# Roman-HLIS-Cosmology-PIT/romanimpreprocess

Measured on AMD Instinct MI355X. Metric: SCA ramps/sec (4096x4096x8grp full L1->L2 chain), higher is better.
Workload: dtype f32

## Files before the change

### romanimpreprocess_amd/csrc/chain2_form.h

```cpp
#pragma once
#include "rip_common.h"

constexpr int c2_block(int n, int want) {
    int d = want < 1 ? 1 : want;
    while (n % d) --d;
    return d;
}
template <int G, bool K64>
struct C2Form {
    static_assert(G % 2 == 0 && G > 4 && G <= 16, "forms exist for whole pairs of groups, 6 to 16");
    static constexpr int narrow = G > 8 ? 2 : (K64 ? 1 : 0);
    static constexpr int cols = (narrow == 0 || (narrow == 2 && K64)) ? 256 : 384;
    static constexpr int threads = 2 * cols;
    static constexpr int outw = cols - 4;
    static constexpr int nstrips(int nx) { return (nx - 4 + outw - 1) / outw < 1 ? 1 : (nx - 4 + outw - 1) / outw; }
    static constexpr int wps = narrow == 0 ? 4 : ((narrow == 2 && K64) ? 2 : 3);

    static constexpr int ks = K64 ? 8 : 4;
    static constexpr int x_ofs = 0;
    static constexpr int o1_ofs = x_ofs + G / 2 * 3 * cols * 8;
    static constexpr int dq_ofs = o1_ofs + G * 3 * cols * ks;
    static constexpr bool wring = narrow < 2;
    static constexpr int qs_ofs = dq_ofs + 3 * cols * 4;
    static constexpr int gn_ofs = qs_ofs + (wring ? 3 * ((G + 3) / 4) * cols * 4 : 0);
    static constexpr int nlc = cols / RIP_CW + 1;
    static constexpr int ln_ofs = gn_ofs + (wring ? 3 * cols * 4 : 0);
    static constexpr int kr_ofs = ln_ofs + nlc * G * 2 * 8;
    static constexpr int krn_room = (160 * 1024 - kr_ofs) / (2 * cols * ks);
    static constexpr int krn = narrow == 2 ? 0 : (krn_room < 9 ? krn_room : 9);
    static constexpr int lds_bytes = kr_ofs + 2 * krn * cols * ks;
    static_assert(lds_bytes <= (narrow == 0 ? 80 : 160) * 1024, "the 256-column form runs two workgroups per CU, the others one");

    static constexpr int stream_aux = narrow == 2 ? 2 : 0;
    static constexpr int pb = c2_block(G / 2, narrow == 2 ? (K64 ? 4 : 1) : 2);
    static constexpr int pbc = c2_block(G / 2, wps == 2 ? 2 : 1);
    static constexpr int nbo = c2_block(G, G > 8 ? 4 : 2);
    static_assert((G / 2) % pb == 0 && (G / 2) % pbc == 0 && G % nbo == 0, "block factors divide their counts");
};

static inline long chain2_geometry(ChainArgs &a, int nstrips, int live_last, int slots, int reserve, int wc = 4, bool quad_ok = true) {
    const int maxr = (a.ny + 7) / 8;
    auto cdiv = [](int x, int y) { return (x + y - 1) / y; };
    int best_nr = 0, best_nq = 0, best_steps = 1 << 30;
    if (quad_ok && nstrips > 1 && live_last <= 64) {
        const int nfull = nstrips - 1;
        for (int pass = 0; pass < 2 && !best_nr; ++pass) {
            const int avail = slots - (pass ? 0 : reserve);
            for (int nq = 1; wc * nq <= maxr && nq < avail; ++nq) {
                int nr = (avail - nq) / nfull;
                if (nr > maxr) nr = maxr;
                if (nr < 1) break;
                const int steps = cdiv(a.ny, nr) > cdiv(a.ny, wc * nq) ? cdiv(a.ny, nr) : cdiv(a.ny, wc * nq);
                if (steps < best_steps) best_steps = steps, best_nr = nr, best_nq = nq;
            }
        }
    }
    int nr_u = (slots - reserve) / nstrips;
    if (nr_u < 1) nr_u = slots / nstrips;
    if (nr_u > maxr) nr_u = maxr;
    if (nr_u < 1) nr_u = 1;
    if (best_nr && best_steps < cdiv(a.ny, nr_u)) {
        a.geo_nr = best_nr, a.geo_rows = cdiv(a.ny, best_nr), a.geo_nq = best_nq, a.geo_rows_q = cdiv(a.ny, wc * best_nq);
        return (long)best_nr * (nstrips - 1) + best_nq;
// ... 20 lines not shown
```

### romanimpreprocess_amd/csrc/chain2_kernel.h

```cpp
#pragma once
#include "chain_common.h"
#include "chain2_form.h"

#if (defined(C2_DBG) || defined(CH_STAMP)) && !defined(RIP_TIMING_BUILD)
#error "C2_DBG / CH_STAMP are timing experiments: build them with -DRIP_TIMING_BUILD"
#endif
#ifdef CH_STAMP
#define C2_DRAIN()                                \
    if (a.dbg & 2048) {                           \
        __builtin_amdgcn_s_waitcnt(0);            \
    }
#else
#define C2_DRAIN()
#endif
#define C2_SYNC() __syncthreads()

__device__ __forceinline__ unsigned c2_opaque(unsigned x) {
    asm volatile("" : "+v"(x));
    return x;
}

__device__ __forceinline__ __amdgpu_buffer_rsrc_t c2_rsrc(const void *p, int records = -1) {
    return __builtin_amdgcn_make_buffer_rsrc(const_cast<void *>(p), 0, records, 0x00020000);
}
// ... 58 lines not shown
    static_assert(NA >= NG && G0 >= 0 && G0 < NG, "the values G0 .. NG - 1 of NA are divided");
    const double b = (double)bf;
    double y = __builtin_amdgcn_rcp(b);
    double e = __builtin_fma(-b, y, 1.0);
    y = __builtin_fma(y, e, y);
    e = __builtin_fma(-b, y, 1.0);
    y = __builtin_fma(y, e, y);
    float asum = 0.0f, amin = 3.0e38f;
#pragma unroll
    for (int g = G0; g < NG; ++g) {
        const double q0 = a[g] * y;
        const double r = __builtin_fma(-b, q0, a[g]);
        qf[g] = (float)__builtin_fma(r, y, q0);
        asum = asum + fabsf(qf[g]);
        amin = fminf(amin, fabsf(qf[g]));
    }
    const bool ok = rcp_safe(bf) && asum < 5.7e17f && amin > 1.8e-18f;
    if (!__all(ok || !use)) {
#pragma unroll
        for (int g = G0; g < NG; ++g) qf[g] = (float)(a[g] / b);
    }
}

template <int NP>
struct C2Legendre {
    const float (&cfs)[NP], (&c1s)[NP], (&c2s)[NP], (&chfs)[NP];
    static constexpr __device__ int n() { return NP; }
    __device__ __forceinline__ float cf(int L) const { return cfs[L]; }
    __device__ __forceinline__ float c1(int L) const { return c1s[L]; }
    __device__ __forceinline__ float c2(int L) const { return c2s[L]; }
    __device__ __forceinline__ float chf(int L) const { return chfs[L]; }
};

template <int NP, int G, int START, typename KT, bool SKIP0 = false>
__global__ __launch_bounds__((C2Form<G + (G & 1), sizeof(KT) == 8>::threads), (C2Form<G + (G & 1), sizeof(KT) == 8>::wps)) void chain2_kernel(
    ChainArgs a, const RipPlanHeader *__restrict__ h, const RipVariant *__restrict__ vars, const float *__restrict__ kvals,
    const RipDiff *__restrict__ diffs, double guard) {
    static_assert(G > 4 && G <= 16, "pairs of groups; the groupdq bytes travel packed four to a word");
    static_assert(!SKIP0 || START == 1, "group 0 can be skipped only where the fit excludes it");
    constexpr int GE = G + (G & 1);
    using F = C2Form<GE, sizeof(KT) == 8>;
    constexpr int COLS = F::cols;
    constexpr int KRN = F::krn;
    constexpr bool KFIT = F::narrow > 0;
    constexpr int QW = (G + 3) / 4;
    constexpr int GP = GE / 2;
    static_assert(QW == (GE + 3) / 4, "the padded count packs into the same flag words");
    constexpr bool K64 = sizeof(KT) == 8;
    constexpr int SA = F::stream_aux;
    extern __shared__ __align__(16) unsigned char lds_raw[];
    constexpr int XR = 3;
    f2 *X2 = reinterpret_cast<f2 *>(lds_raw + F::x_ofs);
    f2 *O12 = reinterpret_cast<f2 *>(lds_raw + F::o1_ofs);
    double *O1d = reinterpret_cast<double *>(lds_raw + F::o1_ofs);
    uint32_t *DQ = reinterpret_cast<uint32_t *>(lds_raw + F::dq_ofs);
    uint32_t *QS = reinterpret_cast<uint32_t *>(lds_raw + F::qs_ofs);
    float *GN = reinterpret_cast<float *>(lds_raw + F::gn_ofs);
    double *LN = reinterpret_cast<double *>(lds_raw + F::ln_ofs);
    constexpr int NLC = F::nlc;
    f2 *KR2 = reinterpret_cast<f2 *>(lds_raw + F::kr_ofs);
    float *KR1 = reinterpret_cast<float *>(KR2 + 2 * 4 * COLS);
    double *KRd = reinterpret_cast<double *>(lds_raw + F::kr_ofs);

    const RIP_K C2KernArgs *kargs = (const RIP_K C2KernArgs *)__builtin_amdgcn_kernarg_segment_ptr();
    const int tid = threadIdx.x;
    if (a.wg_counter && tid == 0) __hip_atomic_fetch_add(a.wg_counter, 1u, __ATOMIC_RELAXED, __HIP_MEMORY_SCOPE_AGENT);
#ifdef C2_DBG
    const int dbg = a.dbg;
#else
    constexpr int dbg = 0;
#endif
    const bool fit_role = tid >= COLS;
    const int col = fit_role ? tid - COLS : tid;
    const int ny = a.ny, nx = a.nx, nb = a.nb;
    const int ay0 = nb, ay1 = ny - nb, ax0 = nb, ax1 = nx - nb;
    const unsigned npix = (unsigned)ny * (unsigned)nx;
    const unsigned pl4 = npix * 4u;
    const int nch = nx / RIP_CW;
    const uint32_t bad = DQ_NO_LIN_CORR | DQ_REFERENCE_PIXEL;

    float c1[NP], c2[NP], chf[NP];
#pragma unroll
    for (int L = 1; L < NP; ++L) {
        const RipLegendreK k = rip_legendre_k(L);
        c1[L] = k.c1, c2[L] = k.c2, chf[L] = k.chf;
    }

    const int nstrips = F::nstrips(nx);
    const int bid = c2_xcd_block((int)blockIdx.x, (int)gridDim.x);
    const int nfull = a.geo_rows_q ? nstrips - 1 : nstrips;
    const bool quad = bid >= nfull * a.geo_nr;
// ... 59 lines not shown
            rok[dyi] = sy >= ay0 && sy < ay1;
            rowoff[dyi] = (unsigned)min(max(sy, ylo), yhi) * (row4 * ES);
        }
        const unsigned rowbits = rip_ipc_row_mask(rok[0], rok[1], rok[2]);
        const __amdgpu_buffer_rsrc_t kr = c2_rsrc(kern_base);
        unsigned pofs = 0;
#pragma unroll
        for (int p = 0; p < 9; ++p) {
            const int dy = p / 3 - 1, dx = p % 3 - 1;
            const int k = rip_ipc_term(dy, dx);
            if constexpr (PAIRS) {
                const float kv_ = c2_ld_f32(kr, cx4[dx + 1], pofs + rowoff[dy + 1]);
                if (k & 1)
                    kk[k / 2].y = kv_;
                else
                    kk[k / 2].x = kv_;
            } else {
                if (k >= KMIN) kk[k] = c2_ld_f64(kr, cx4[dx + 1] * 2u, pofs + rowoff[dy + 1]);
            }
            pofs += pl4 * ES;
        }
        const unsigned um = (want && y >= ay0 && y < ay1) ? rowbits : 0u;
        return lane_mask & um;
    };
    auto k_valid = [&](int y) -> unsigned {
        const bool r0 = (y + 1) >= ay0 && (y + 1) < ay1, r1 = y >= ay0 && y < ay1, r2 = (y - 1) >= ay0 && (y - 1) < ay1;
        return r1 ? (lane_mask & rip_ipc_row_mask(r0, r1, r2)) : 0u;
    };
#ifdef CH_STAMP
    unsigned long long st_[9] = {0, 0, 0, 0, 0, 0, 0, 0, 0};
    unsigned long long tl_ = __builtin_amdgcn_s_memtime();
#endif
    if (!fit_role) {
        auto fetch_groups = [&](const RIP_K ChainArgs *ka, int y, int g0, int g1, RowRegs<NP, GE> &rr) {
            if ((dbg & 64) && y > R0 - 2) return;
            __builtin_amdgcn_sched_barrier(0);
            const unsigned yl = (unsigned)min(max(y, ylo), yhi);
            const __amdgpu_buffer_rsrc_t rs = c2_rsrc(ka->data), rq = c2_rsrc(ka->gdq), rd = c2_rsrc(ka->dark_data),
                                         rb = c2_rsrc(ka->bias, ka->bias_records);
            unsigned o4 = yl * row4 + (unsigned)g0 * pl4, o2 = yl * (row4 >> 1) + (unsigned)g0 * (pl4 >> 1),
                     o1 = yl * (row4 >> 2) + (unsigned)g0 * npix;
#pragma unroll
            for (int g = g0; g < g1; ++g) {
                if constexpr (GE > G) {
                    if (g >= G) continue;
                }
                const bool flags_only = SKIP0 && g == 0;
                if (!flags_only) rr.S[g] = c2_ld_u16<SA>(rs, cc2, o2);
                rr.q[g] = c2_ld_u8<F::wring ? SA : 0>(rq, cc1, o1);
                if (!flags_only) {
                    rr.dk[g] = c2_ld_f32<SA>(rd, cc4, o4);
                    rr.bs[g] = c2_ld_f32<SA>(rb, cc4, o4);
                }
                o4 += pl4;
                o2 += pl4 >> 1;
                o1 += npix;
            }
            __builtin_amdgcn_sched_barrier(0);
        };
        auto fetch_coefs = [&](const RIP_K ChainArgs *ka, int y, int i0, int i1, RowRegs<NP, GE> &rr) {
            if ((dbg & 64) && y > R0 - 2) return;
            __builtin_amdgcn_sched_barrier(0);
            const unsigned yl = (unsigned)min(max(y, ylo), yhi);
            const __amdgpu_buffer_rsrc_t rp = c2_rsrc(ka->planes);
            unsigned o4 = yl * row4 + (unsigned)i0 * pl4;
#pragma unroll
            for (int i = i0; i < i1; ++i) {
                if (i < NP)
                    rr.cf[i] = c2_ld_f32<SA>(rp, cc4, o4);
                else if (i == NP)
                    rr.smin = c2_ld_f32<SA>(rp, cc4, o4);
                else if (i == NP + 1)
                    rr.smax = c2_ld_f32<SA>(rp, cc4, o4);
                else if (i == NP + 2)
                    rr.sref = c2_ld_f32<SA>(rp, cc4, o4);
                else if (i == NP + 3)
                    rr.dq = c2_ld_u32<SA>(rp, cc4, yl * row4 + (unsigned)(NP + ka->merged_dq) * pl4);
                else
                    rr.gain = c2_ld_f32<F::wring ? SA : 0>(rp, cc4, o4);
                o4 += pl4;
            }
            __builtin_amdgcn_sched_barrier(0);
        };
        auto fetch_row = [&](int y, RowRegs<NP, GE> &rr) {
            const RIP_K ChainArgs *ka = &kargs->a;
            fetch_coefs(ka, y, 0, NP + 5, rr);
            fetch_groups(ka, y, 0, G, rr);
        };
        constexpr int NCO = NP + 5;
        constexpr int CO_STEP = (NCO + GP - 1) / GP;
        RowRegs<NP, GE> rr;
        if constexpr (GE > G) rr.S[G] = rr.q[G] = 0u, rr.dk[G] = rr.bs[G] = 0.0f;
        if constexpr (SKIP0) rr.S[0] = 0u, rr.dk[0] = rr.bs[0] = 0.0f;
        fetch_row(R0 - 2, rr);
        int so_c = (R0 - 5 + 2 + 3000) % 3;
        double rcn[G];
        {
            const RIP_K double *rt = rip_k(kargs->a.rowcorr_t) + (size_t)min(max(R0 - 2, 0), ny - 1) * G;
#pragma unroll
            for (int g = SKIP0 ? 1 : 0; g < G; ++g) rcn[g] = rt[g];
            if constexpr (SKIP0) rcn[0] = 0.0;
        }
        for (int r = R0 - 5; r <= R0 + rows_wg; ++r, so_c = (so_c == 2) ? 0 : so_c + 1) {
            const RIP_K ChainArgs *ka = &c2_args(kargs)->a;
            const int yi = r + 3, yc = r + 2;
            const bool do_a = (yi >= R0 - 2) && (yi <= R1 + 1);
            const bool do_c = (yc >= R0 - 1) && (yc <= R1);
            double rc[G];
#pragma unroll
            for (int g = 0; g < G; ++g) rc[g] = rcn[g];
            {
                const RIP_K double *rt = rip_k(ka->rowcorr_t) + (size_t)min(max(yi + 1, 0), ny - 1) * G;
#pragma unroll
                for (int g = SKIP0 ? 1 : 0; g < G; ++g) rcn[g] = rt[g];
            }
            const bool a_full = do_a && yi >= 0 && yi < ny;
            const int xslot = (so_c == 2) ? 0 : so_c + 1;
            f2 *xs = X2 + xslot * COLS + col;
            const bool act = col_act && yi >= ay0 && yi < ay1;
            uint32_t dq = rr.dq;
            uint32_t w[QW];
#pragma unroll
            for (int i = 0; i < QW; ++i) w[i] = 0;
            const float smin = rr.smin;
            const float span = rr.smax - smin;
            const bool fastdiv = __all(rcp_safe(span));
            const float rspan = rip_rcp_mid(span);
            const double yd = (double)yi;
            constexpr int PB = F::pb;
#pragma unroll
            for (int pb = 0; pb < GP; pb += PB) {
                f2 zz[PB], SS[PB];
                bool any_ex = false;
                if (a_full && !(dbg & 32)) {
                    f2 tt[PB], quo[PB];
#pragma unroll
                    for (int b = 0; b < PB; ++b) {
                        const int p = pb + b;
                        float Sv[2];
#pragma unroll
                        for (int e = 0; e < 2; ++e) {
                            const int g = 2 * p + e;
                            if constexpr (GE > G) {
                                if (g >= G) {
                                    Sv[e] = Sv[0];
                                    continue;
                                }
                            }
                            if constexpr (SKIP0) {
                                if (g == 0) {
                                    w[0] |= rr.q[0] & 0xffu;
                                    continue;
                                }
                            }
                            const double *ln = LN + (chr * G + g) * 2;
                            float S = rip_refpix_apply((float)rr.S[g], rr.dk[g], rc[g], ln[0], ln[1], yd);
                            if (act) S = S - rr.bs[g];
                            Sv[e] = S;
                            w[g / 4] |= (rr.q[g] & 0xffu) << (8 * (g & 3));
                        }
                        if constexpr (SKIP0) {
                            if (p == 0) Sv[0] = Sv[1];
                        }
                        SS[b] = f2{Sv[0], Sv[1]};
                        const f2 t = SS[b] - f2{smin, smin};
                        tt[b] = t * 2.0f;
                    }
                    if (fastdiv) {
#pragma unroll
                        for (int b = 0; b < PB; ++b) quo[b] = div_rcp2(tt[b], span, rspan);
                    } else {
#pragma unroll
                        for (int b = 0; b < PB; ++b) quo[b] = f2{tt[b].x / span, tt[b].y / span};
                    }
#pragma unroll
                    for (int b = 0; b < PB; ++b) {
                        f2 z = quo[b] + (-1.0f);
                        if constexpr (!SKIP0) {
                            if (pb + b == 0 && a.do_not_flag_first) z.x = clip2<float>(z.x, -1.0f, 1.0f);
                        }
                        zz[b] = z;
                        any_ex = any_ex || (fabsf(z.x) > 1.0f) || (fabsf(z.y) > 1.0f);
                    }
                } else {
#pragma unroll
                    for (int b = 0; b < PB; ++b) zz[b] = SS[b] = f2{0.0f, 0.0f};
                }
                fetch_groups(ka, r + 4, 2 * pb, 2 * (pb + PB), rr);
                if (a_full && (dbg & 16)) {
#pragma unroll
// ... 74 lines not shown
                        if constexpr (SKIP0) {
                            if (p == 0) xv.x = 0.0f;
                        }
                        xs[p * XR * COLS] = col_ok ? xv : f2{0.0f, 0.0f};
                    }
                } else if (do_a) {
#pragma unroll
                    for (int b = 0; b < PB; ++b) xs[(pb + b) * XR * COLS] = f2{0.0f, 0.0f};
                }
            }
            if (do_a) {
                const bool keep = a_full && col_ok;
                DQ[xslot * COLS + col] = keep ? dq : 0u;
                if constexpr (F::wring) {
#pragma unroll
                    for (int i = 0; i < QW; ++i) QS[(xslot * QW + i) * COLS + col] = keep ? w[i] : 0u;
                    GN[xslot * COLS + col] = rr.gain;
                }
            }
            f2 kC[5];
            double kCd[9];
            kC[4].y = 0.0f;
            unsigned vC;
            if constexpr (K64)
                vC = load_k(ka->kern, yc, do_c && wcol >= 1 && wcol < wl - 1, kCd, C2Int<0>{});
            else
                vC = load_k(ka->kern, yc, do_c && wcol >= 1 && wcol < wl - 1, kC, C2Int<0>{});
            CH_T(2)
            C2_SYNC();
            CH_T(3)
            const RIP_K ChainArgs *kb2 = &c2_args(kargs)->a;
            auto fetch_coefs_beside = [&](int p) { fetch_coefs(kb2, r + 4, p * CO_STEP, min(p * CO_STEP + CO_STEP, NCO), rr); };
            CH_T(4)
            {
                const bool all = __all(vC == 0x1ffu || vC == 0u);
                const int so = so_c;
                const int sm = (so == 0) ? 2 : so - 1, s0 = so, sp = (so == 2) ? 0 : so + 1;
                if constexpr (KRN > 0) {
                    const int ks = yc & 1;
                    if constexpr (K64) {
#pragma unroll
                        for (int k = 0; k < KRN; ++k) KRd[(ks * KRN + k) * COLS + col] = kCd[k];
                    } else {
#pragma unroll
                        for (int i = 0; i < 4; ++i) KR2[(ks * 4 + i) * COLS + col] = kC[i];
                        KR1[ks * COLS + col] = kC[4].x;
                    }
                }
                if constexpr (K64) {
                    constexpr int PBC = F::pbc;
#pragma unroll
                    for (int p0 = 0; p0 < GP; p0 += PBC) {
#pragma unroll
                        for (int q = 0; q < PBC; ++q)
                            fetch_coefs_beside(p0 + q);
                        if (do_c) {
                            float v[2 * PBC][9];
#pragma unroll
                            for (int q = 0; q < PBC; ++q) {
                                const f2 *xb = X2 + (p0 + q) * XR * COLS + col;
                                const f2 *xm_ = xb + sm * COLS, *x0_ = xb + s0 * COLS, *xp_ = xb + sp * COLS;
                                const f2 tt[9] = {x0_[0], xm_[0], xp_[0], x0_[-1], x0_[1], xm_[-1], xm_[1], xp_[-1], xp_[1]};
#pragma unroll
                                for (int k = 0; k < 9; ++k) v[2 * q][k] = tt[k].x, v[2 * q + 1][k] = tt[k].y;
                            }
                            double f[2 * PBC];
// ... 318 lines not shown
                    for (int i = 0; i < QW; ++i) qw_next[i] = QS[(sn * QW + i) * COLS + col];
                    gain_next = GN[sn * COLS + col];
                } else {
                    const unsigned yl = (unsigned)min(max((dbg & 1024) ? R0 : r + 1, ylo), yhi);
                    const __amdgpu_buffer_rsrc_t rq = c2_rsrc(kg->a.gdq);
                    unsigned o1 = yl * (row4 >> 2);
#pragma unroll
                    for (int g = 0; g < G; ++g) {
                        qb_next[g] = c2_ld_u8(rq, cc1, o1);
                        o1 += npix;
                    }
                    gain_next = c2_ld_f32(c2_rsrc(kg->a.planes), cc4, (unsigned)(NP + 4) * pl4 + yl * row4);
                }
            }
            if constexpr (KFIT) {
                if constexpr (K64)
                    (void)load_k(kg->a.kern, (dbg & 1024) ? R0 : r + 1, true, kn_d, C2Int<KRN>{});
                else
                    (void)load_k(kg->a.kern, (dbg & 1024) ? R0 : r + 1, true, kn, C2Int<0>{});
            }
            CH_T(6)
            C2_SYNC();
            CH_T(7)
        }
    }
#ifdef CH_STAMP
    if ((tid & 63) == 0 && a.dbg_buf) {
        unsigned long long *o = a.dbg_buf + ((size_t)blockIdx.x * (F::threads / 64) + (tid >> 6)) * 9;
        for (int i = 0; i < 9; ++i) o[i] += st_[i];
    }
#endif
}

template <int NP, int G, int START, typename KT, bool SKIP0 = false>
static int launch_chain2_s(rip_ctx *ctx, const RipPlan *plan, const ChainArgs &a) {
    using F = C2Form<G + (G & 1), sizeof(KT) == 8>;
    const size_t lds = F::lds_bytes;
    if (a.nb < 2) return 1;
    ChainArgs ag = a;
    const long grid = c2_form_geometry<F>(ag, ctx->ncu, ctx->chain_reserve, ctx->chain_quad, ctx->last_geo);
    static bool lds_set[64] = {};
    if (lds > 48 * 1024 && !lds_set[ctx->device & 63]) {
        RIP_HIP(ctx, hipFuncSetAttribute(reinterpret_cast<const void *>(chain2_kernel<NP, G, START, KT, SKIP0>),
                                         hipFuncAttributeMaxDynamicSharedMemorySize, (int)lds));
        lds_set[ctx->device & 63] = true;
    }
    hipLaunchKernelGGL((chain2_kernel<NP, G, START, KT, SKIP0>), dim3((unsigned)grid), dim3(F::threads), lds, ctx->stream, ag,
                       reinterpret_cast<const RipPlanHeader *>(plan->dev), plan->d_variants, plan->d_k, plan->d_diffs,
                       ctx->guard_band);
    RIP_HIP(ctx, hipGetLastError());
    if (ag.wg_counter) ctx->gate_total += (uint32_t)grid, ctx->gate_armed = true;
    return RIP_OK;
}

template <int NP, int G, typename KT>
static int launch_chain2(rip_ctx *ctx, const RipPlan *plan, const ChainArgs &a, bool skip0) {
    if (plan->h.start == 0 && plan->dense.valid == rip_full_valid<G, 0>()) return skip0 ? 1 : launch_chain2_s<NP, G, 0, KT>(ctx, plan, a);
    if (plan->h.start == 1 && plan->dense.valid == rip_full_valid<G, 1>())
        return skip0 ? launch_chain2_s<NP, G, 1, KT, true>(ctx, plan, a) : launch_chain2_s<NP, G, 1, KT>(ctx, plan, a);
    return 1;
}

template <int NP, typename KT, int PART>
int rip_launch_chain2(rip_ctx *ctx, const RipPlan *plan, const ChainArgs &a, bool skip0) {
    static_assert(PART >= 0 && PART <= 2, "parts of RIP_CHAIN_G_ALL");
#define C2_CASE(g) \
    if (a.ngrp == g) return launch_chain2<NP, g, KT>(ctx, plan, a, skip0);
    if constexpr (PART == 0) {
        RIP_CHAIN_G_PART0(C2_CASE)
    } else if constexpr (PART == 1) {
        RIP_CHAIN_G_PART1(C2_CASE)
    } else {
        RIP_CHAIN_G_PART2(C2_CASE)
    }
#undef C2_CASE
    return 1;
}
```

### romanimpreprocess_amd/csrc/chain_common.h

```cpp
#pragma once
#include "rip_common.h"

#include "device_rampfit.h"

#ifdef CH_STAMP
#define CH_T(i)                                                     \
    {                                                               \
        const unsigned long long t_ = __builtin_amdgcn_s_memtime(); \
        __builtin_amdgcn_s_waitcnt(0xC07F);                         \
        st_[i] += t_ - tl_;                                         \
        tl_ = t_;                                                   \
    }
#else
#define CH_T(i)
#endif

typedef float f2 __attribute__((ext_vector_type(2)));

__device__ __forceinline__ f2 div_rcp2(f2 a, float b, float rb) {
    const f2 nb = {-b, -b}, rr = {rb, rb};
    const f2 q0 = a * rr;
    const f2 r0 = __builtin_elementwise_fma(nb, q0, a);
    const f2 q1 = __builtin_elementwise_fma(r0, rr, q0);
    const f2 r1 = __builtin_elementwise_fma(nb, q1, a);
// ... 12 lines not shown
    f2 v[NB][9];
    __builtin_amdgcn_sched_barrier(0);
#pragma unroll
    for (int b = 0; b < NB; ++b) {
        v[b][5] = rm[b][t - 1];
        v[b][1] = rm[b][t];
        v[b][6] = rm[b][t + 1];
        v[b][3] = r0[b][t - 1];
        v[b][0] = r0[b][t];
        v[b][4] = r0[b][t + 1];
        v[b][7] = rp[b][t - 1];
        v[b][2] = rp[b][t];
        v[b][8] = rp[b][t + 1];
    }
    __builtin_amdgcn_sched_barrier(0);
    f2 acc[NB];
#pragma unroll
    for (int b = 0; b < NB; ++b) acc[b] = v[b][0] * RIP_KSPLAT(kk2, 0);
#pragma unroll
    for (int k = 1; k < 9; ++k) {
#pragma unroll
        for (int b = 0; b < NB; ++b) {
            const f2 p = v[b][k] * RIP_KSPLAT(kk2, k);
            acc[b] = (ALL || ((valid >> k) & 1u)) ? acc[b] + p : acc[b];
        }
    }
#pragma unroll
    for (int b = 0; b < NB; ++b) {
        f[b] = acc[b];
        ctr[b] = v[b][0];
    }
}

template <int NP, int G>
struct RowRegs {
    uint32_t S[G];
    uint32_t q[G];
    float dk[G], bs[G];
    float cf[NP], smin, smax, sref, gain;
    uint32_t dq;
};
```

### romanimpreprocess_amd/csrc/device_rampfit.h

```cpp
#pragma once
#include "rip_common.h"

#define RIP_K __attribute__((address_space(4)))
template <typename T>
__device__ __forceinline__ const RIP_K T *rip_k(const T *p) {
    return (const RIP_K T *)p;
}
#define KLD(x) (*rip_k(&(x)))
__device__ __forceinline__ RipVariant rip_load_variant(const RipVariant *vars, int i) {
    RipVariant v;
    v.g = KLD(vars[i].g);
    v.ndiff = KLD(vars[i].ndiff);
    v.diff_ofs = KLD(vars[i].diff_ofs);
    v.k_ofs = KLD(vars[i].k_ofs);
    v.coef = KLD(vars[i].coef);
    v.rfac = KLD(vars[i].rfac);
    return v;
}

__device__ __forceinline__ float log_f32(float x) {
    return (float)log((double)x);
}

__device__ __forceinline__ float hypot_f32(float a, float b) {
// ... 23 lines not shown
    return fmaf(r1, rb, q1);
}
__device__ __forceinline__ float rip_sqrt_mid(float x) {
    const float s = __builtin_amdgcn_sqrtf(x);
    const float sd = __uint_as_float(__float_as_uint(s) - 1u), su = __uint_as_float(__float_as_uint(s) + 1u);
    const float rd = fmaf(-sd, s, x), ru = fmaf(-su, s, x);
    float r = (rd <= 0.0f) ? sd : s;
    r = (ru > 0.0f) ? su : r;
    return r;
}

template <typename T>
__device__ __forceinline__ T clip_lo(T x, T lo) {
    return x < lo ? lo : x;
}
template <typename T>
__device__ __forceinline__ T clip2(T x, T lo, T hi) {
    return x < lo ? lo : (x > hi ? hi : x);
}

template <typename GT>
struct GainConst;
template <>
struct GainConst<float> {
    static __device__ __forceinline__ float lo() { return 1e-4f; }
    static __device__ __forceinline__ float hi() { return 1e4f; }
};
template <>
struct GainConst<double> {
    static __device__ __forceinline__ double lo() { return 1e-4; }
    static __device__ __forceinline__ double hi() { return 1e4; }
};

__device__ __forceinline__ float rip_refpix_apply(float S, float dk, double rc, double m, double c, double yd) {
    float v = S - dk;
    v = (float)((double)v - rc);
    const double iel = m * yd + c;
    v = (float)((double)v - iel);
    return v + dk;
}

struct RipLegendreK {
    float c1, c2, chf;
};
__device__ __forceinline__ RipLegendreK rip_legendre_k(int L) {
    RipLegendreK k;
    k.c1 = (float)((double)(2 * L + 1) / (double)(L + 1));
    k.c2 = (float)((double)L / (double)(L + 1));
    k.chf = (float)((double)(L * (L + 1)) / 2.0);
    return k;
}

template <typename T>
__device__ __forceinline__ float rip_legendre_series(float z, const T tab, bool &ex) {
    const float az = fabsf(z);
    ex = az > 1.0f;
    const float exc = az - 1.0f;
    const bool neg = z < 0.0f;
    float phi = tab.cf(0);
    float pp = 1.0f, pc = z;
    for (int L = 1; L < tab.n(); ++L) {
        float e = 1.0f + tab.chf(L) * exc;
        e = (neg && (L & 1)) ? -e : e;
        const float sel = ex ? e : pc;
        const float term = tab.cf(L) * sel;
        phi = phi + term;
        const float u = tab.c1(L) * z;
        const float pn = u * pc - tab.c2(L) * pp;
        pp = pc;
        pc = pn;
    }
    return phi;
// ... 269 lines not shown
                    hit = (double)sme > sth;
                }
            }
            if (hit && flag) jmask |= 1u << i;
        }
    }
}

typedef float rf2 __attribute__((ext_vector_type(2)));

struct RipFitConst {
    float ia, ib;
    float sa32;
    float slope_th;
    float inv_ia;
};
__device__ __forceinline__ RipFitConst rip_fit_const(const RipPlanHeader *h) {
    RipFitConst c;
    c.ia = KLD(h->ia);
    c.ib = KLD(h->ib);
    c.sa32 = (float)KLD(h->sa);
    c.slope_th = (float)(KLD(h->dsb) / KLD(h->loglen));
    c.inv_ia = 1.0f / c.ia;
    return c;
}

__device__ __forceinline__ void rip_load_pair(RipDensePair &r, const RipDense *dn, int ps) {
#pragma unroll
    for (int e = 0; e < 2; ++e) {
        r.inv_dt[e] = KLD(dn->pairs[ps].inv_dt[e]);
        r.A[e] = KLD(dn->pairs[ps].A[e]);
        r.B[e] = KLD(dn->pairs[ps].B[e]);
        r.k1[e] = KLD(dn->pairs[ps].k1[e]);
    }
}

template <int G, int START>
constexpr uint32_t rip_full_valid() {
    return rip_full_valid_of(G, START);
}

struct RipFitState {
    float s, er, ep;
    float dv, s2, xc;
    uint32_t jfast, unsure;
    bool live;
};

template <int G, uint32_t VALID = 0u, bool SKIP0 = false>
__device__ __forceinline__ void fit_full_pk_a(const rf2 (&dA)[(G + 1) / 2], const RipFitConst fc, const RipVariant v,
                                              const RipDense *__restrict__ dn, float gain, float rn, bool flag, double guard,
                                              RipFitState &st) {
    constexpr int GP = (G + 1) / 2;
    constexpr int NS = 2 * GP;
    float k2[G];
#pragma unroll
    for (int t = 0; t < G; ++t) k2[t] = KLD(dn->K2[t]);
    const uint32_t valid = VALID ? VALID : KLD(dn->valid);
    RipDensePair tab[2];
    rip_load_pair(tab[0], dn, 0);
    const float d1 = dA[0].y;
    const rf2 d11 = {d1, d1};
    float s = 0.0f;
#pragma unroll
    for (int p = 0; p < GP; ++p) {
        const rf2 diff = dA[p] - d11;
// ... 11 lines not shown
                continue;
            }
        }
        const rf2 kk = {k2[2 * p], k2[2 * p + 1]};
        const rf2 prod = kk * diff;
        s = s + prod.x;
        s = s + prod.y;
    }
    float dv;
    rip_slope_errors<float, true>(s, gain, rn, v, dv, st.er, st.ep);
    st.s = s;
    st.dv = dv;
    st.s2 = rn * rn;
    st.jfast = 0;
    st.unsure = 0;
    st.xc = 0.0f;
    st.live = __any(flag);
    if (!st.live) return;

    const float xc = clip2<float>(s, fc.ia, fc.ib);
    st.xc = xc;
    const bool need_log = xc != fc.ia;
    float lx = 0.0f;
    if (__any(need_log)) lx = need_log ? __logf(xc * fc.inv_ia) : 0.0f;
    const float slope_th = fc.slope_th;
    const float sth32 = fc.sa32 + slope_th * lx;
    const float band0 = 2e-6f * fabsf(sth32) + 4.5e-6f * fabsf(slope_th) + 1e-30f;
    const float s2 = st.s2;
    const float s8 = fabsf(s) * 8.1e-7f;
    const float thp = sth32 + band0, thm = sth32 - band0;
    const float rsmax = __frsqrt_rn(KLD(dn->amin) * s2) * 1.000001f;
    const bool pass = fmaf(s8, rsmax, band0) <= 0.5f * sth32;
    const bool lane_exact = !(guard < 1e300) || !pass;
    uint32_t jfast = 0, unsure_mask = 0;
    rf2 dB[GP];
#pragma unroll
    for (int p = 0; p < GP; ++p) dB[p] = rf2{dA[p].y, (p + 1 < GP) ? dA[p + 1].x : 0.0f};
#pragma unroll
    for (int ps = 0; ps < NS; ++ps) {
        if (ps + 1 < NS) rip_load_pair(tab[(ps + 1) & 1], dn, ps + 1);
        const int ip = ps / 2, di = (ps & 1) + 1;
        const uint32_t vbits = (valid >> (2 * ps)) & 3u;
        if (vbits == 0) continue;
        const rf2 hi = (di == 1) ? dB[ip] : ((ip + 1 < GP) ? dA[ip + 1] : rf2{0.0f, 0.0f});
        const rf2 lo = dA[ip];
        const RipDensePair &r = tab[ps & 1];
        const rf2 num = hi - lo;
        const rf2 q = num * rf2{r.inv_dt[0], r.inv_dt[1]};
        const rf2 delta = q - rf2{s, s};
        const rf2 as2 = rf2{r.A[0], r.A[1]} * s2;
        const rf2 var = __builtin_elementwise_fma(rf2{r.B[0], r.B[1]}, rf2{dv, dv}, as2);
        const rf2 rs = {__frsqrt_rn(var.x), __frsqrt_rn(var.y)};
        const rf2 sm = delta * rs;
        const rf2 t = rs * s8;
        const rf2 k1 = {r.k1[0], r.k1[1]};
        const rf2 hiT = (t + thp) * k1;
        const rf2 loT = (rf2{thm, thm} - t) * (rf2{2.0f, 2.0f} - k1);
#pragma unroll
        for (int e = 0; e < 2; ++e) {
            if (!((vbits >> e) & 1u)) continue;
            const float sme = e ? sm.y : sm.x;
            const bool hit = sme > (e ? hiT.y : hiT.x);
            const bool nohit = sme < (e ? loT.y : loT.x);
            if (hit) jfast |= 1u << (2 * ps + e);
            if (lane_exact || !(hit || nohit)) unsure_mask |= 1u << (2 * ps + e);
        }
    }
    st.jfast = jfast;
    st.unsure = unsure_mask;
}

template <int G>
__device__ __forceinline__ void fit_full_pk_b(const rf2 (&dA)[(G + 1) / 2], const RipPlanHeader *__restrict__ h,
                                              const RipFitConst fc, const RipDense *__restrict__ dn,
                                              const float *__restrict__ kv, const RipDiff *__restrict__ df, bool flag,
                                              const RipFitState &st, uint32_t &jmask) {
    constexpr int GP = (G + 1) / 2;
    if (!st.live) return;
    const float s = st.s, dv = st.dv, s2 = st.s2, xc = st.xc;
    uint32_t jfast = st.jfast;
    const uint32_t unsure_mask = st.unsure;
    if (__any(unsure_mask != 0 && flag)) {
        const double sth = rip_exact_sth<true>(xc, fc.ia, h);
        for (int bit = 0; bit < 4 * GP; ++bit) {
            if (!__any((unsure_mask >> bit) & 1u)) continue;
            if ((unsure_mask >> bit) & 1u) {
                const RipDiff rd = df[KLD(dn->kidx[bit])];
                float di_ = 0.0f, dj_ = 0.0f;
#pragma unroll
                for (int p = 0; p < GP; ++p) {
// ... 89 lines not shown
```

### romanimpreprocess_amd/csrc/plan.hip

```cpp
#include <string.h>

#include <cmath>
#include <memory>

#include "rip_host.h"

static std::vector<float> variant_weights(const rip_plan_desc *d, int v, int g, int start) {
    std::vector<float> K(g, 0.0f);
    if (v == 0) {
        for (int i = 0; i < g; ++i) K[i] = d->K[i];
    } else {
        K[g - 1] = 1.0f / (d->tbar[g - 1] - d->tbar[start]);
        K[start] = -K[g - 1];
    }
    return K;
}

extern "C" {

int rip_plan_desc_first_weight_zero(const rip_plan_desc *d) {
    if (!d || !d->exclude_first || d->ngrp < 3 || d->ngrp > RIP_MAX_GROUPS) return 0;
    const int G = d->ngrp, nvar = 1 + (G - 4 > 0 ? G - 4 : 0);
    for (int v = 0; v < nvar; ++v)
        if (variant_weights(d, v, v == 0 ? G : G - v, 1)[0] != 0.0f) return 0;
// ... 71 lines not shown
    const size_t o_var = al(sizeof(RipPlanHeader));
    const size_t o_k = o_var + al(p->variants.size() * sizeof(RipVariant));
    const size_t o_d = o_k + al(p->kvals.size() * sizeof(float));
    const size_t o_dense = o_d + al(p->diffs.size() * sizeof(RipDiff));
    p->bytes = o_dense + al(sizeof(RipDense));
    {
        RipDense &dn = p->dense;
        memset(&dn, 0, sizeof dn);
        for (int i = 0; i < G; ++i) dn.K2[i] = d->K[i];
        const RipVariant &v0 = p->variants[0];
        double amin = 1e301;
        for (int k = 0; k < v0.ndiff; ++k) {
            const RipDiff &df = p->diffs[v0.diff_ofs + k];
            const int i = df.i, di = df.j - df.i, ps = 2 * (i / 2) + (di - 1), e = i & 1;
            if (G <= 16) dn.valid |= 1u << (2 * ps + e);
            dn.kidx[2 * ps + e] = k;
            dn.pairs[ps].inv_dt[e] = df.inv_dt;
            dn.pairs[ps].A[e] = df.A;
            dn.pairs[ps].B[e] = df.B;
            const double r = (double)df.relerr + 4.1e-7;
            if (r < 9.9e-3) {
                dn.pairs[ps].k1[e] = std::nextafter((float)((1.0 / (1.0 - r)) * (1.0 + 4e-7)), INFINITY);
            } else {
                dn.pairs[ps].k1[e] = INFINITY;
            }
            amin = (df.B >= 0.0f) ? std::fmin(amin, (double)df.A) : 0.0;
        }
        dn.amin = (v0.ndiff > 0 && amin > 0.0 && amin < 1e300) ? (float)(amin * (1.0 - 1e-6)) : 0.0f;
        for (int ps = 0; ps < RIP_MAX_GROUPS; ++ps)
            for (int e = 0; e < 2; ++e) {
                const int bit = 2 * ps + e;
                const bool used = bit < 32 && ((dn.valid >> bit) & 1u);
                if (!used) dn.pairs[ps].A[e] = 1.0f;
            }
    }
    p->k0_zero = rip_plan_desc_first_weight_zero(d) == 1;
    std::vector<char> img(p->bytes, 0);
    memcpy(img.data(), &h, sizeof h);
    memcpy(img.data() + o_var, p->variants.data(), p->variants.size() * sizeof(RipVariant));
    memcpy(img.data() + o_k, p->kvals.data(), p->kvals.size() * sizeof(float));
    if (!p->diffs.empty()) memcpy(img.data() + o_d, p->diffs.data(), p->diffs.size() * sizeof(RipDiff));
    memcpy(img.data() + o_dense, &p->dense, sizeof(RipDense));
    hipError_t e = hipMalloc(&p->dev, p->bytes);
    if (e == hipSuccess) e = hipMemcpy(p->dev, img.data(), p->bytes, hipMemcpyHostToDevice);
    if (e != hipSuccess) return rip_fail(ctx, RIP_EHIP, "plan upload: %s", hipGetErrorString(e));
    p->d_variants = reinterpret_cast<const RipVariant *>((char *)p->dev + o_var);
    p->d_k = reinterpret_cast<const float *>((char *)p->dev + o_k);
    p->d_diffs = reinterpret_cast<const RipDiff *>((char *)p->dev + o_d);
    p->d_dense = reinterpret_cast<const RipDense *>((char *)p->dev + o_dense);
    int id = -1;
    for (size_t i = 0; i < ctx->plans.size(); ++i)
        if (!ctx->plans[i]) {
            id = (int)i;
            break;
        }
    if (id < 0) {
        ctx->plans.push_back(nullptr);
        id = (int)ctx->plans.size() - 1;
    }
    ctx->plans[id] = p.release();
    *plan_id = id;
    return RIP_OK;
}

int rip_plan_destroy(rip_ctx *ctx, int id) {
    if (id < 0 || id >= (int)ctx->plans.size() || !ctx->plans[id]) return rip_fail(ctx, RIP_EINVAL, "plan %d does not exist", id);
// ... 16 lines not shown
```

### romanimpreprocess_amd/csrc/rip_common.h

```cpp
#pragma once

#include <hip/hip_runtime.h>
#include <stdint.h>

#include <string>
#include <map>
#include <vector>

#include "../../include/romanhip.h"

#define DQ_DO_NOT_USE 0x1u
#define DQ_SATURATED 0x2u
#define DQ_JUMP_DET 0x4u
#define DQ_NO_FLAT_FIELD (1u << 18)
#define DQ_NO_GAIN_VALUE (1u << 19)
#define DQ_NO_LIN_CORR (1u << 20)
#define DQ_REFERENCE_PIXEL (1u << 31)

#define RIP_CW RIP_CHANNEL_WIDTH

struct RipDiff {
    int32_t i, j;
    float dt;
    float A, B;
    float inv_dt;
    float relerr;
    float pad_[1];
};

struct RipVariant {
    int32_t g;
    int32_t ndiff, diff_ofs, k_ofs;
    float coef, rfac;
};

struct RipPlanHeader {
    int32_t ngrp, start, nvariants, do_not_flag_first;
    double sa, dsb;
    double loglen;
    float ia, ib;
    float tbar[RIP_MAX_GROUPS], tau[RIP_MAX_GROUPS], nreads[RIP_MAX_GROUPS];
};

struct RipDensePair {
    float inv_dt[2], A[2], B[2];
    float k1[2];
};
struct RipDense {
    uint32_t valid;
    int32_t kidx[2 * RIP_MAX_GROUPS];
    float amin;
    float K2[RIP_MAX_GROUPS];
    RipDensePair pairs[RIP_MAX_GROUPS];
};

constexpr uint32_t rip_full_valid_of(int G, int start) {
    uint32_t m = 0;
    for (int i = start; i < G - 1; ++i) {
        const int dimax = (i == G - 2 || G - 1 - start == 2) ? 1 : 2;
        for (int di = 1; di <= dimax; ++di) m |= 1u << (2 * (2 * (i / 2) + (di - 1)) + (i & 1));
    }
    return m;
}

struct RipPlan {
    RipPlanHeader h;
    std::vector<RipVariant> variants;
    std::vector<float> kvals;
    std::vector<RipDiff> diffs;
    void *dev = nullptr;
    const RipVariant *d_variants = nullptr;
    const float *d_k = nullptr;
    const RipDiff *d_diffs = nullptr;
    const RipDense *d_dense = nullptr;
    RipDense dense;
    size_t bytes = 0;
    bool k0_zero = false;
};

// ... 277 lines not shown
```

Baseline: 1288.

## Drop bias stream when absent, table ref-pixel lines per row, precompute jump thresholds

New measurement: 1325, median of 6. +2.9%, better.

```diff
diff --git a/romanimpreprocess_amd/csrc/chain2_form.h b/romanimpreprocess_amd/csrc/chain2_form.h
--- a/romanimpreprocess_amd/csrc/chain2_form.h
+++ b/romanimpreprocess_amd/csrc/chain2_form.h
@@ -28,7 +28,10 @@
     static constexpr int kr_ofs = ln_ofs + nlc * G * 2 * 8;
     static constexpr int krn_room = (160 * 1024 - kr_ofs) / (2 * cols * ks);
     static constexpr int krn = narrow == 2 ? 0 : (krn_room < 9 ? krn_room : 9);
-    static constexpr int lds_bytes = kr_ofs + 2 * krn * cols * ks;
+    static constexpr bool nobias = narrow == 0;
+    static constexpr bool lt = narrow == 0;
+    static constexpr int lt_ofs = kr_ofs + 2 * krn * cols * ks;
+    static constexpr int lds_bytes = lt_ofs + (lt ? (cols / 64) * nlc * G * 8 : 0);
     static_assert(lds_bytes <= (narrow == 0 ? 80 : 160) * 1024, "the 256-column form runs two workgroups per CU, the others one");
 
     static constexpr int stream_aux = narrow == 2 ? 2 : 0;
diff --git a/romanimpreprocess_amd/csrc/chain2_kernel.h b/romanimpreprocess_amd/csrc/chain2_kernel.h
--- a/romanimpreprocess_amd/csrc/chain2_kernel.h
+++ b/romanimpreprocess_amd/csrc/chain2_kernel.h
@@ -114,7 +114,7 @@
     __device__ __forceinline__ float chf(int L) const { return chfs[L]; }
 };
 
-template <int NP, int G, int START, typename KT, bool SKIP0 = false>
+template <int NP, int G, int START, typename KT, bool SKIP0 = false, bool BIAS = true>
 __global__ __launch_bounds__((C2Form<G + (G & 1), sizeof(KT) == 8>::threads), (C2Form<G + (G & 1), sizeof(KT) == 8>::wps)) void chain2_kernel(
     ChainArgs a, const RipPlanHeader *__restrict__ h, const RipVariant *__restrict__ vars, const float *__restrict__ kvals,
     const RipDiff *__restrict__ diffs, double guard) {
@@ -122,6 +122,8 @@
     static_assert(!SKIP0 || START == 1, "group 0 can be skipped only where the fit excludes it");
     constexpr int GE = G + (G & 1);
     using F = C2Form<GE, sizeof(KT) == 8>;
+    static_assert(BIAS || F::nobias, "only the forms the table names have an instantiation without a bias stream");
+    constexpr bool LT = F::lt;
     constexpr int COLS = F::cols;
     constexpr int KRN = F::krn;
     constexpr bool KFIT = F::narrow > 0;
@@ -139,6 +141,7 @@
     uint32_t *QS = reinterpret_cast<uint32_t *>(lds_raw + F::qs_ofs);
     float *GN = reinterpret_cast<float *>(lds_raw + F::gn_ofs);
     double *LN = reinterpret_cast<double *>(lds_raw + F::ln_ofs);
+    double *LTB = reinterpret_cast<double *>(lds_raw + F::lt_ofs);
     constexpr int NLC = F::nlc;
     f2 *KR2 = reinterpret_cast<f2 *>(lds_raw + F::kr_ofs);
     float *KR1 = reinterpret_cast<float *>(KR2 + 2 * 4 * COLS);
@@ -264,7 +267,7 @@
     unsigned long long tl_ = __builtin_amdgcn_s_memtime();
 #endif
     if (!fit_role) {
-        auto fetch_groups = [&](const RIP_K ChainArgs *ka, int y, int g0, int g1, RowRegs<NP, GE> &rr) {
+        auto fetch_groups = [&](const RIP_K ChainArgs *ka, int y, int g0, int g1, RowRegs<NP, GE, BIAS> &rr) {
             if ((dbg & 64) && y > R0 - 2) return;
             __builtin_amdgcn_sched_barrier(0);
             const unsigned yl = (unsigned)min(max(y, ylo), yhi);
@@ -282,7 +285,7 @@
                 rr.q[g] = c2_ld_u8<F::wring ? SA : 0>(rq, cc1, o1);
                 if (!flags_only) {
                     rr.dk[g] = c2_ld_f32<SA>(rd, cc4, o4);
-                    rr.bs[g] = c2_ld_f32<SA>(rb, cc4, o4);
+                    if constexpr (BIAS) rr.bs[g] = c2_ld_f32<SA>(rb, cc4, o4);
                 }
                 o4 += pl4;
                 o2 += pl4 >> 1;
@@ -290,7 +293,7 @@
             }
             __builtin_amdgcn_sched_barrier(0);
         };
-        auto fetch_coefs = [&](const RIP_K ChainArgs *ka, int y, int i0, int i1, RowRegs<NP, GE> &rr) {
+        auto fetch_coefs = [&](const RIP_K ChainArgs *ka, int y, int i0, int i1, RowRegs<NP, GE, BIAS> &rr) {
             if ((dbg & 64) && y > R0 - 2) return;
             __builtin_amdgcn_sched_barrier(0);
             const unsigned yl = (unsigned)min(max(y, ylo), yhi);
@@ -314,17 +317,34 @@
             }
             __builtin_amdgcn_sched_barrier(0);
         };
-        auto fetch_row = [&](int y, RowRegs<NP, GE> &rr) {
+        auto fetch_row = [&](int y, RowRegs<NP, GE, BIAS> &rr) {
             const RIP_K ChainArgs *ka = &kargs->a;
             fetch_coefs(ka, y, 0, NP + 5, rr);
             fetch_groups(ka, y, 0, G, rr);
         };
         constexpr int NCO = NP + 5;
         constexpr int CO_STEP = (NCO + GP - 1) / GP;
-        RowRegs<NP, GE> rr;
-        if constexpr (GE > G) rr.S[G] = rr.q[G] = 0u, rr.dk[G] = rr.bs[G] = 0.0f;
-        if constexpr (SKIP0) rr.S[0] = 0u, rr.dk[0] = rr.bs[0] = 0.0f;
+        RowRegs<NP, GE, BIAS> rr;
+        if constexpr (GE > G) rr.S[G] = rr.q[G] = 0u, rr.dk[G] = 0.0f;
+        if constexpr (SKIP0) rr.S[0] = 0u, rr.dk[0] = 0.0f;
+        if constexpr (BIAS) {
+            if constexpr (GE > G) rr.bs[G] = 0.0f;
+            if constexpr (SKIP0) rr.bs[0] = 0.0f;
+        }
         fetch_row(R0 - 2, rr);
+        const int lt_lane = tid & 63;
+        double *lt_w = LTB + (tid >> 6) * (NLC * GE);
+        auto line_values = [&](int y) {
+            if constexpr (LT) {
+                static_assert(NLC * GE <= 64, "one lane per (channel, group) of the wave's table");
+                if (lt_lane < NLC * GE) {
+                    const int ch = lt_lane / GE, g = lt_lane % GE;
+                    const double *ln = LN + (ch * G + (g < G ? g : 0)) * 2;
+                    lt_w[lt_lane] = rip_refpix_line(ln[0], ln[1], (double)y);
+                }
+            }
+        };
+        line_values(R0 - 2);
         int so_c = (R0 - 5 + 2 + 3000) % 3;
         double rcn[G];
         {
@@ -385,9 +405,16 @@
                                     continue;
                                 }
                             }
-                            const double *ln = LN + (chr * G + g) * 2;
-                            float S = rip_refpix_apply((float)rr.S[g], rr.dk[g], rc[g], ln[0], ln[1], yd);
-                            if (act) S = S - rr.bs[g];
+                            float S;
+                            if constexpr (LT) {
+                                S = rip_refpix_apply_iel((float)rr.S[g], rr.dk[g], rc[g], lt_w[chr * GE + g]);
+                            } else {
+                                const double *ln = LN + (chr * G + g) * 2;
+                                S = rip_refpix_apply((float)rr.S[g], rr.dk[g], rc[g], ln[0], ln[1], yd);
+                            }
+                            if constexpr (BIAS) {
+                                if (act) S = S - rr.bs[g];
+                            }
                             Sv[e] = S;
                             w[g / 4] |= (rr.q[g] & 0xffu) << (8 * (g & 3));
                         }
@@ -528,6 +555,7 @@
             const RIP_K ChainArgs *kb2 = &c2_args(kargs)->a;
             auto fetch_coefs_beside = [&](int p) { fetch_coefs(kb2, r + 4, p * CO_STEP, min(p * CO_STEP + CO_STEP, NCO), rr); };
             CH_T(4)
+            line_values(r + 4);
             {
                 const bool all = __all(vC == 0x1ffu || vC == 0u);
                 const int so = so_c;
@@ -912,7 +940,7 @@
 #endif
 }
 
-template <int NP, int G, int START, typename KT, bool SKIP0 = false>
+template <int NP, int G, int START, typename KT, bool SKIP0 = false, bool BIAS = true>
 static int launch_chain2_s(rip_ctx *ctx, const RipPlan *plan, const ChainArgs &a) {
     using F = C2Form<G + (G & 1), sizeof(KT) == 8>;
     const size_t lds = F::lds_bytes;
@@ -921,11 +949,11 @@
     const long grid = c2_form_geometry<F>(ag, ctx->ncu, ctx->chain_reserve, ctx->chain_quad, ctx->last_geo);
     static bool lds_set[64] = {};
     if (lds > 48 * 1024 && !lds_set[ctx->device & 63]) {
-        RIP_HIP(ctx, hipFuncSetAttribute(reinterpret_cast<const void *>(chain2_kernel<NP, G, START, KT, SKIP0>),
+        RIP_HIP(ctx, hipFuncSetAttribute(reinterpret_cast<const void *>(chain2_kernel<NP, G, START, KT, SKIP0, BIAS>),
                                          hipFuncAttributeMaxDynamicSharedMemorySize, (int)lds));
         lds_set[ctx->device & 63] = true;
     }
-    hipLaunchKernelGGL((chain2_kernel<NP, G, START, KT, SKIP0>), dim3((unsigned)grid), dim3(F::threads), lds, ctx->stream, ag,
+    hipLaunchKernelGGL((chain2_kernel<NP, G, START, KT, SKIP0, BIAS>), dim3((unsigned)grid), dim3(F::threads), lds, ctx->stream, ag,
                        reinterpret_cast<const RipPlanHeader *>(plan->dev), plan->d_variants, plan->d_k, plan->d_diffs,
                        ctx->guard_band);
     RIP_HIP(ctx, hipGetLastError());
@@ -933,12 +961,20 @@
     return RIP_OK;
 }
 
+template <int NP, int G, typename KT, bool BIAS>
+static int launch_chain2_b(rip_ctx *ctx, const RipPlan *plan, const ChainArgs &a, bool skip0) {
+    if (plan->h.start == 0 && plan->dense.valid == rip_full_valid<G, 0>())
+        return skip0 ? 1 : launch_chain2_s<NP, G, 0, KT, false, BIAS>(ctx, plan, a);
+    if (plan->h.start == 1 && plan->dense.valid == rip_full_valid<G, 1>())
+        return skip0 ? launch_chain2_s<NP, G, 1, KT, true, BIAS>(ctx, plan, a) : launch_chain2_s<NP, G, 1, KT, false, BIAS>(ctx, plan, a);
+    return 1;
+}
 template <int NP, int G, typename KT>
 static int launch_chain2(rip_ctx *ctx, const RipPlan *plan, const ChainArgs &a, bool skip0) {
-    if (plan->h.start == 0 && plan->dense.valid == rip_full_valid<G, 0>()) return skip0 ? 1 : launch_chain2_s<NP, G, 0, KT>(ctx, plan, a);
-    if (plan->h.start == 1 && plan->dense.valid == rip_full_valid<G, 1>())
-        return skip0 ? launch_chain2_s<NP, G, 1, KT, true>(ctx, plan, a) : launch_chain2_s<NP, G, 1, KT>(ctx, plan, a);
-    return 1;
+    if constexpr (C2Form<G + (G & 1), sizeof(KT) == 8>::nobias) {
+        if (a.bias_records == 0) return launch_chain2_b<NP, G, KT, false>(ctx, plan, a, skip0);
+    }
+    return launch_chain2_b<NP, G, KT, true>(ctx, plan, a, skip0);
 }
 
 template <int NP, typename KT, int PART>
diff --git a/romanimpreprocess_amd/csrc/chain_common.h b/romanimpreprocess_amd/csrc/chain_common.h
--- a/romanimpreprocess_amd/csrc/chain_common.h
+++ b/romanimpreprocess_amd/csrc/chain_common.h
@@ -68,11 +68,17 @@
     }
 }
 
-template <int NP, int G>
-struct RowRegs {
+template <int G, bool BIAS>
+struct RowBias {
+    float bs[G];
+};
+template <int G>
+struct RowBias<G, false> {};
+template <int NP, int G, bool BIAS = true>
+struct RowRegs : RowBias<G, BIAS> {
     uint32_t S[G];
     uint32_t q[G];
-    float dk[G], bs[G];
+    float dk[G];
     float cf[NP], smin, smax, sref, gain;
     uint32_t dq;
 };
diff --git a/romanimpreprocess_amd/csrc/device_rampfit.h b/romanimpreprocess_amd/csrc/device_rampfit.h
--- a/romanimpreprocess_amd/csrc/device_rampfit.h
+++ b/romanimpreprocess_amd/csrc/device_rampfit.h
@@ -79,12 +79,15 @@
     static __device__ __forceinline__ double hi() { return 1e4; }
 };
 
-__device__ __forceinline__ float rip_refpix_apply(float S, float dk, double rc, double m, double c, double yd) {
+__device__ __forceinline__ double rip_refpix_line(double m, double c, double yd) { return m * yd + c; }
+__device__ __forceinline__ float rip_refpix_apply_iel(float S, float dk, double rc, double iel) {
     float v = S - dk;
     v = (float)((double)v - rc);
-    const double iel = m * yd + c;
     v = (float)((double)v - iel);
     return v + dk;
+}
+__device__ __forceinline__ float rip_refpix_apply(float S, float dk, double rc, double m, double c, double yd) {
+    return rip_refpix_apply_iel(S, dk, rc, rip_refpix_line(m, c, yd));
 }
 
 struct RipLegendreK {
@@ -420,6 +423,7 @@
         r.A[e] = KLD(dn->pairs[ps].A[e]);
         r.B[e] = KLD(dn->pairs[ps].B[e]);
         r.k1[e] = KLD(dn->pairs[ps].k1[e]);
+        r.k2[e] = KLD(dn->pairs[ps].k2[e]);
     }
 }
 
@@ -497,6 +501,8 @@
     const float rsmax = __frsqrt_rn(KLD(dn->amin) * s2) * 1.000001f;
     const bool pass = fmaf(s8, rsmax, band0) <= 0.5f * sth32;
     const bool lane_exact = !(guard < 1e300) || !pass;
+    const float tmax = s8 * rsmax;
+    const float hp = thp + tmax, lm = thm - tmax;
     uint32_t jfast = 0, unsure_mask = 0;
     rf2 dB[GP];
 #pragma unroll
@@ -517,10 +523,8 @@
         const rf2 var = __builtin_elementwise_fma(rf2{r.B[0], r.B[1]}, rf2{dv, dv}, as2);
         const rf2 rs = {__frsqrt_rn(var.x), __frsqrt_rn(var.y)};
         const rf2 sm = delta * rs;
-        const rf2 t = rs * s8;
-        const rf2 k1 = {r.k1[0], r.k1[1]};
-        const rf2 hiT = (t + thp) * k1;
-        const rf2 loT = (rf2{thm, thm} - t) * (rf2{2.0f, 2.0f} - k1);
+        const rf2 hiT = rf2{hp, hp} * rf2{r.k1[0], r.k1[1]};
+        const rf2 loT = rf2{lm, lm} * rf2{r.k2[0], r.k2[1]};
 #pragma unroll
         for (int e = 0; e < 2; ++e) {
             if (!((vbits >> e) & 1u)) continue;
diff --git a/romanimpreprocess_amd/csrc/plan.hip b/romanimpreprocess_amd/csrc/plan.hip
--- a/romanimpreprocess_amd/csrc/plan.hip
+++ b/romanimpreprocess_amd/csrc/plan.hip
@@ -127,6 +127,7 @@
                 const int bit = 2 * ps + e;
                 const bool used = bit < 32 && ((dn.valid >> bit) & 1u);
                 if (!used) dn.pairs[ps].A[e] = 1.0f;
+                dn.pairs[ps].k2[e] = 2.0f - dn.pairs[ps].k1[e];
             }
     }
     p->k0_zero = rip_plan_desc_first_weight_zero(d) == 1;
diff --git a/romanimpreprocess_amd/csrc/rip_common.h b/romanimpreprocess_amd/csrc/rip_common.h
--- a/romanimpreprocess_amd/csrc/rip_common.h
+++ b/romanimpreprocess_amd/csrc/rip_common.h
@@ -45,6 +45,7 @@
 struct RipDensePair {
     float inv_dt[2], A[2], B[2];
     float k1[2];
+    float k2[2];
 };
 struct RipDense {
     uint32_t valid;
```
